# zengxiaofei/HapHiC

Hardware: AMD Instinct MI355X
Metric: Hi-C pairs/s ingested (link-matrix build) + MCL iters/s (higher is better)
Workload: dtype u64 keys + u32 counts (ingest); f32 values, exact u64 fixed-point accumulation (MCL)

## Files before the change

haphic_amd/csrc/hhx_ingest.h:

```cpp
#pragma once
#include "hhx_common.h"
#include "hhx_internal.h"

namespace hhx {

constexpr int ID_BITS = 29;
constexpr u64 ID_MASK = (1ull << ID_BITS) - 1;
constexpr u64 KEY_MASK = (1ull << (2 * ID_BITS)) - 1;
constexpr int HT_SHIFT = 58;
constexpr u64 FULL_BIT = 1ull << 60, FLANK_BIT = 1ull << 61;
constexpr u64 EMPTY_KEY = ~0ull, NO_ORD = ~0ull;

struct LinkRun {
    i64 n = 0;
    DevBuf<u64> key, ord_full, ord_flank;
    DevBuf<u32> ht;
    DevBuf<u32> fl;
    bool has_stats = false;
    unsigned long long stats[3] = {0, 0, 0};
    int alloc(i64 rows) {
        n = rows;
        return key.alloc((size_t)rows) || ord_full.alloc((size_t)rows) || ord_flank.alloc((size_t)rows) ||
               ht.alloc((size_t)rows * 4) || fl.alloc((size_t)rows);
    }
// ... 84 lines not shown
    bool ready = false;
    i64 n_full = 0, n_flank = 0;
    DevBuf<i32> full_i, full_j, flank_i, flank_j;
    DevBuf<i64> full_cnt, ht, flank_cnt;
    DevBuf<double> flank_val;
    DevBuf<unsigned long long> frag_links;
};

}

struct hhx_ingest {
    hhx::DevTables t{};
    hhx::DevBuf<hhx::UnitInfo> ctg_info, frag_info;
    bool combined = true;
    u64 ord_base = 0;
    u64 n_pushed = 0;
    u64 ord_limit = 0;
    std::vector<hhx::LinkRun *> runs[3];
    bool keep_frag_pairs = false;
    bool finalized = false;
    i64 n_full = 0, n_flank = 0;
    hhx::OrderedTables ordered;
    bool keep_pairs = false;
    std::vector<hhx::DevBuf<u64>> side_key, side_xy;
    i64 n_side = 0;
    bool links_dropped = false;
    std::vector<i32> frag_ctg;
    bool pairs_dropped = false;
    i64 max_ctg_len = 0;
    hhx::DevBuf<i32> stage[4];
    hhx::DevBuf<i64> stage64[2];
    ~hhx_ingest() {
        for (auto &v : runs)
            for (auto *r : v) delete r;
    }
    const hhx::LinkRun *table(int which) const {
        const auto &v = runs[(combined || which == 0) ? 0 : 1];
        return v.empty() ? nullptr : v[0];
    }
};

template <class POS>
int hhx_side_records_push(hhx_ingest *h, i64 n_pairs, const i32 *id1, const POS *pos1, const i32 *id2, const POS *pos2);

namespace hhx {
struct PairGroups {
    i64 K = 0, N = 0;
    DevBuf<u64> skey, sxy, stk, srank;
    DevBuf<i64> gstart;
};
int group_pairs(hhx_ingest *h, PairGroups &G, const char *who);
}

int hhx_link_matrix_from_run(const hhx::LinkRun *run, i32 n_frag, u64 ord_limit, const uint8_t *in_set_host, i32 n_rest, int add_self_loops,
                             i32 *frag_index_host, i32 *n_linked_out, hhx_csr **out);

namespace hhx {
int ingest_write_clm_fd(hhx_ingest *h, int fd, const uint8_t *names_blob, const i64 *name_off, i64 *n_lines, i64 *n_bytes);
}
```

haphic_amd/csrc/hhx_ingest.hip:

```cpp
#include "hhx_ingest.h"
#include "hhx_partition.h"

using namespace hhx;

namespace {

__device__ __host__ __forceinline__ u64 mix64(u64 x) {
    x ^= x >> 33; x *= 0xff51afd7ed558ccdULL; x ^= x >> 33; x *= 0xc4ceb9fe1a85ec53ULL; x ^= x >> 33;
    return x;
}
__device__ __forceinline__ u32 bucket_of(u64 key, int total_bits) {
    return total_bits ? (u32)(mix64(key) >> (64 - total_bits)) : 0u;
}

template <bool COMBINED, class POS = i32>
struct SrcPairs {
    typedef u32 w1_t;
    static constexpr bool MARK = false;
    static constexpr bool BATCHED = false;
    const i32 *id1; const POS *pos1; const i32 *id2; const POS *pos2;
    DevTables t;
    int stream;
    __device__ __forceinline__ bool get(i64 idx, u64 &rec, u32 &ord) const {
        ord = (u32)idx;
// ... 763 lines not shown
    if (key) *key = r ? r->key.p : nullptr;
    if (ord_full) *ord_full = r ? r->ord_full.p : nullptr;
    if (ord_flank) *ord_flank = r ? r->ord_flank.p : nullptr;
    if (ht) *ht = r ? r->ht.p : nullptr;
    if (flank) *flank = r ? r->fl.p : nullptr;
    return 0;
}

extern "C" int hhx_ingest_fetch(hhx_ingest *h, i32 *full_i, i32 *full_j, i64 *full_cnt, i64 *ht_cnt, i32 *flank_i, i32 *flank_j,
                                i64 *flank_cnt, i64 *frag_links) {
    if (!h || !h->finalized) return fail("ingest handle not finalized");
    HHX_TRY(materialize(h));
    const OrderedTables &o = h->ordered;
    const size_t nf = (size_t)o.n_full, nk = (size_t)o.n_flank;
    if (full_i && nf) HHX_HIP(hipMemcpyAsync(full_i, o.full_i.p, 4 * nf, hipMemcpyDeviceToHost, g_stream));
    if (full_j && nf) HHX_HIP(hipMemcpyAsync(full_j, o.full_j.p, 4 * nf, hipMemcpyDeviceToHost, g_stream));
    if (full_cnt && nf) HHX_HIP(hipMemcpyAsync(full_cnt, o.full_cnt.p, 8 * nf, hipMemcpyDeviceToHost, g_stream));
    if (ht_cnt && nf) HHX_HIP(hipMemcpyAsync(ht_cnt, o.ht.p, 32 * nf, hipMemcpyDeviceToHost, g_stream));
    if (flank_i && nk) HHX_HIP(hipMemcpyAsync(flank_i, o.flank_i.p, 4 * nk, hipMemcpyDeviceToHost, g_stream));
    if (flank_j && nk) HHX_HIP(hipMemcpyAsync(flank_j, o.flank_j.p, 4 * nk, hipMemcpyDeviceToHost, g_stream));
    if (flank_cnt && nk) HHX_HIP(hipMemcpyAsync(flank_cnt, o.flank_cnt.p, 8 * nk, hipMemcpyDeviceToHost, g_stream));
    if (frag_links) HHX_HIP(hipMemcpyAsync(frag_links, o.frag_links.p, 8 * (size_t)h->t.n_frag, hipMemcpyDeviceToHost, g_stream));
    HHX_HIP(hipStreamSynchronize(g_stream));
    return 0;
}

int hhx_ingest_ordered_full_device(hhx_ingest *h, const i32 **fi, const i32 **fj) {
    HHX_TRY(materialize(h));
    *fi = h->ordered.full_i.p;
    *fj = h->ordered.full_j.p;
    return 0;
}

extern "C" int hhx_ingest_flank_device(hhx_ingest *h, void **fi, void **fj, void **val) {
    if (!h || !h->finalized) return fail("ingest handle not finalized");
    HHX_TRY(materialize(h));
    if (fi) *fi = h->ordered.flank_i.p;
    if (fj) *fj = h->ordered.flank_j.p;
    if (val) *val = h->ordered.flank_val.p;
    return 0;
}

extern "C" int hhx_ingest_flank_count_device(hhx_ingest *h, void **cnt_i64) {
    if (!h || !h->finalized) return fail("ingest handle not finalized");
    HHX_TRY(materialize(h));
    if (cnt_i64) *cnt_i64 = h->ordered.flank_cnt.p;
    return 0;
}

extern "C" int hhx_ingest_link_matrix(hhx_ingest *h, const uint8_t *in_set_host, int32_t n_rest, int add_self_loops,
                                      int32_t *frag_index_host, int32_t *n_linked, hhx_csr **out) {
    if (!h || !h->finalized) return fail("ingest handle not finalized");
    KTimer kt("link_matrix");
    return hhx_link_matrix_from_run(h->table(1), h->t.n_frag, h->ord_limit, in_set_host, n_rest, add_self_loops, frag_index_host, n_linked, out);
}

extern "C" int hhx_ingest_destroy(hhx_ingest *h) {
    if (h) files_wait_handle(h);
    delete h;
    return 0;
}
```

haphic_amd/csrc/hhx_matrix.hip:

```cpp
#include "hhx_ingest.h"
#include "hhx_partition.h"
#include "hhx_sort.h"

using namespace hhx;

namespace {

struct RowsView {
    const i32 *fi, *fj;
    const double *val;
    __device__ __forceinline__ bool get(i64 k, i32 &a, i32 &b, u64 &ord, float &v) const {
        a = fi[k]; b = fj[k]; ord = (u64)k;
        v = (float)val[k];
        return true;
    }
};
struct RunView {
    const u64 *key, *ord_flank;
    const u32 *fl;
    __device__ __forceinline__ bool get(i64 k, i32 &a, i32 &b, u64 &ord, float &v) const {
        ord = ord_flank[k];
        if (ord == NO_ORD) return false;
        a = (i32)(key[k] >> ID_BITS); b = (i32)(key[k] & ID_MASK);
        v = (float)fl[k];
// ... 213 lines not shown
namespace {

struct SrcDirected {
    typedef u64 w1_t;
    static constexpr bool MARK = false;
    static constexpr bool BATCHED = false;
    const u64 *key, *ord_flank;
    const u32 *fl;
    const unsigned char *in_set;
    __device__ __forceinline__ bool get(i64 idx, u64 &w0, u64 &w1) const {
        const i64 k = idx >> 1;
        const u64 ord = ord_flank[k];
        if (ord == NO_ORD) return false;
        const u64 ky = key[k];
        const u32 i = (u32)(ky >> ID_BITS), j = (u32)(ky & ID_MASK);
        if (!in_set[i] || !in_set[j]) return false;
        const u32 side = (u32)(idx & 1);
        const u32 a = side ? j : i, b = side ? i : j;
        w0 = ((u64)a << ID_BITS) | (u64)b;
        w1 = ((2 * ord + side) << 31) | (u64)fl[k];
        return true;
    }
};
struct DigRow {
    __device__ __forceinline__ u32 operator()(u64 w0) const { return (u32)(w0 >> ID_BITS); }
};

constexpr int PK_ID_BITS = 20, PK_CNT_BITS = 24;
constexpr u32 PK_ID_MASK = (1u << PK_ID_BITS) - 1, PK_CNT_MASK = (1u << PK_CNT_BITS) - 1;
__device__ __forceinline__ u32 xcc_id() {
#if defined(__HIP_DEVICE_COMPILE__)
    return __builtin_amdgcn_s_getreg((3 << 11) | 20) & 7u;
#else
    return 0;
#endif
}
constexpr i32 D2M_LDS_MAX_FRAGS = 1 << 19;
struct PackedRawBase { u64 ord, ky; u32 c; };
struct PackedRawWords : PackedRawBase { u32 wi, wj; };
template <bool IN_LDS>
struct SrcDirectedPacked {
    typedef NoPayload w1_t;
    static constexpr bool MARK = true;
    static constexpr bool BATCHED = true;
    static constexpr bool LDS_TABLE = IN_LDS;
    static constexpr size_t LDS_TABLE_MAX = (size_t)D2M_LDS_MAX_FRAGS / 8;
    static constexpr int CHUNK = 7, CHUNK_SCATTER = 4;
    const u64 *key, *ord_flank;
    const u32 *fl;
    const u32 *in_bits;
    unsigned long long *first_pos;
    unsigned int *too_big;
    i32 n_frag;
    typedef typename std::conditional<IN_LDS, PackedRawBase, PackedRawWords>::type Raw;
    static constexpr int PREFETCH = 1;
    static __device__ __forceinline__ void pin(Raw &r) { asm volatile("" : "+v"(r.ord)); asm volatile("" : "+v"(r.ky)); asm volatile("" : "+v"(r.c)); }
    __device__ __forceinline__ u32 frag_i(const Raw &r) const { return min((u32)(r.ky >> ID_BITS), (u32)n_frag - 1u); }
    __device__ __forceinline__ u32 frag_j(const Raw &r) const { return min((u32)(r.ky & ID_MASK), (u32)n_frag - 1u); }
    size_t lds_table_bytes() const { return ((size_t)n_frag + 31) / 32 * sizeof(u32); }
    __device__ __forceinline__ SrcDirectedPacked lds_table(void *at) const {
        u32 *t = (u32 *)at;
        const u32 words = ((u32)n_frag + 31u) >> 5;
        for (u32 w = threadIdx.x; w < words; w += blockDim.x) t[w] = in_bits[w];
        SrcDirectedPacked s = *this;
        s.in_bits = t;
        return s;
    }
    __device__ __forceinline__ void load1(i64 idx, Raw &r) const {
        const i64 k = idx >> 1;
        r.ord = ord_flank[k]; r.ky = key[k]; r.c = fl[k];
    }
    __device__ __forceinline__ void load2(Raw &r) const {
        if constexpr (!IN_LDS) { r.wi = in_bits[frag_i(r) >> 5]; r.wj = in_bits[frag_j(r) >> 5]; }
    }
    __device__ __forceinline__ bool member(const Raw &r) const {
        const u32 fi = frag_i(r), fj = frag_j(r);
        u32 wi, wj;
        if constexpr (IN_LDS) { wi = in_bits[fi >> 5]; wj = in_bits[fj >> 5]; }
        else { wi = r.wi; wj = r.wj; }
        return ((wi >> (fi & 31u)) & (wj >> (fj & 31u)) & 1u) != 0;
    }
    __device__ __forceinline__ bool decode_marked(i64 idx, const Raw &r, u64 &w0, u64 &extra) const {
        const u32 i = (u32)(r.ky >> ID_BITS), j = (u32)(r.ky & ID_MASK);
        const u32 side = (u32)(idx & 1);
        const u32 a = side ? j : i, b = side ? i : j;
        w0 = ((u64)a << (PK_ID_BITS + PK_CNT_BITS)) | ((u64)b << PK_CNT_BITS) | (u64)(r.c & PK_CNT_MASK);
        extra = r.c > PK_CNT_MASK ? ~0ull : 2 * r.ord + side;
        return r.ord != NO_ORD && member(r);
    }
    __device__ __forceinline__ bool decode(i64 idx, const Raw &r, u64 &w0, NoPayload &) const {
        u64 extra;
        return decode_marked(idx, r, w0, extra);
    }
    __device__ __forceinline__ bool get(i64 idx, u64 &w0, NoPayload &w1) const {
        Raw r;
        load1(idx, r);
        load2(r);
        return decode(idx, r, w0, w1);
    }
    __device__ __forceinline__ unsigned long long *my_table() const {
        return first_pos + (size_t)xcc_id() * (size_t)n_frag;
    }
    __device__ __forceinline__ u64 mark_load(i64 idx, const Raw &r) const {
        if (!first_pos) return 0;
        return __hip_atomic_load(&my_table()[(idx & 1) ? frag_j(r) : frag_i(r)], __ATOMIC_RELAXED, __HIP_MEMORY_SCOPE_AGENT);
    }
    __device__ __forceinline__ void mark_apply(u64 w0, u64 pos, u64 seen) const {
        if (!first_pos) return;
        if (pos == ~0ull) *too_big = 1u;
        else if (pos < seen) atomicMin(&my_table()[(u32)(w0 >> (PK_ID_BITS + PK_CNT_BITS)) & PK_ID_MASK], (unsigned long long)pos);
    }
};
constexpr int N_XCC = 8;
__global__ __launch_bounds__(256) void k_min_over_xcc(i32 n_frag, const unsigned long long *__restrict__ per_xcc, unsigned long long *__restrict__ out) {
    for (i32 f = blockIdx.x * blockDim.x + threadIdx.x; f < n_frag; f += gridDim.x * blockDim.x) {
        unsigned long long m = ~0ull;
#pragma unroll
        for (int x = 0; x < N_XCC; ++x) m = min(m, per_xcc[(size_t)x * n_frag + f]);
        out[f] = m;
    }
}
struct DigRowPacked {
    __device__ __forceinline__ u32 operator()(u64 w0) const { return (u32)(w0 >> (PK_ID_BITS + PK_CNT_BITS)) & PK_ID_MASK; }
};
__global__ __launch_bounds__(256) void k_len_from_base(i32 n_frag, const i64 *__restrict__ base, const i32 *__restrict__ frag_index, i32 *__restrict__ cnt) {
    for (i32 f = blockIdx.x * blockDim.x + threadIdx.x; f < n_frag; f += gridDim.x * blockDim.x)
        if (frag_index[f] >= 0) cnt[frag_index[f]] += (i32)(base[f + 1] - base[f]);
}
__global__ __launch_bounds__(256) void k_iota_u64(i64 n, u64 *out) {
    for (i64 k = (i64)blockIdx.x * blockDim.x + threadIdx.x; k < n; k += (i64)gridDim.x * blockDim.x) out[k] = (u64)k;
}
__global__ __launch_bounds__(256) void k_index_from_sorted(i64 n, const u64 *__restrict__ pos_sorted, const u64 *__restrict__ frag_sorted,
                                                           i32 *__restrict__ frag_index, unsigned int *n_linked) {
    for (i64 k = (i64)blockIdx.x * blockDim.x + threadIdx.x; k < n; k += (i64)gridDim.x * blockDim.x) {
        const bool linked = pos_sorted[k] != ~0ull;
        frag_index[frag_sorted[k]] = linked ? (i32)k : -1;
        if (linked && (k + 1 == n || pos_sorted[k + 1] == ~0ull)) *n_linked = (unsigned int)(k + 1);
    }
}
int rank_first_positions(i32 n_frag, const unsigned long long *first_pos, u64 pos_limit, i32 *frag_index, unsigned int *n_linked_dev) {
    if (n_frag <= 4096) {
        k_rank_first<<<(unsigned)((n_frag + 255) / 256), 256, 0, g_stream>>>(n_frag, first_pos, frag_index, n_linked_dev);
        HHX_LAUNCH_CHECK();
        return 0;
    }
    int bits = 1;
    while (bits < 64 && (pos_limit + 1) >> bits) ++bits;
    DevBuf<u64> iota, ks, vs;
    if (iota.alloc((size_t)n_frag) || ks.alloc((size_t)n_frag) || vs.alloc((size_t)n_frag)) return 1;
    k_iota_u64<<<(unsigned)((n_frag + 255) / 256), 256, 0, g_stream>>>(n_frag, iota.p);
    HHX_LAUNCH_CHECK();
    HHX_TRY(stable_sort_pairs_u64((const u64 *)first_pos, ks.p, iota.p, vs.p, n_frag, bits));
    k_index_from_sorted<<<(unsigned)((n_frag + 255) / 256), 256, 0, g_stream>>>(n_frag, ks.p, vs.p, frag_index, n_linked_dev);
    HHX_LAUNCH_CHECK();
    HHX_HIP(hipStreamSynchronize(g_stream));
    return 0;
}

__global__ __launch_bounds__(256) void k_row_first(i32 n_frag, const i64 *__restrict__ base, const u64 *__restrict__ w1,
                                                   unsigned long long *__restrict__ first_pos, i32 *__restrict__ row_len) {
    const int lane = lane_id();
    for (i32 a = blockIdx.x * 4 + threadIdx.x / HHX_WAVE; a < n_frag; a += gridDim.x * 4) {
        const i64 b = base[a], e = base[a + 1];
        unsigned long long m = ~0ull;
        for (i64 p = b + lane; p < e; p += HHX_WAVE) m = min(m, (unsigned long long)(w1[p] >> 31));
#pragma unroll
        for (int o = 32; o > 0; o >>= 1) m = min(m, (unsigned long long)__shfl_down((long long)m, o, HHX_WAVE));
        if (lane == 0) { first_pos[a] = m; row_len[a] = (i32)(e - b); }
    }
}
__global__ __launch_bounds__(256) void k_len_by_index(i32 n_frag, const i32 *__restrict__ frag_index, const i32 *__restrict__ row_len,
                                                      i32 *__restrict__ cnt) {
    for (i32 f = blockIdx.x * blockDim.x + threadIdx.x; f < n_frag; f += gridDim.x * blockDim.x)
        if (frag_index[f] >= 0) cnt[frag_index[f]] += row_len[f];
}
template <bool PACKED>
__device__ __forceinline__ u32 entry_col(u64 w0) { return PACKED ? ((u32)(w0 >> PK_CNT_BITS) & PK_ID_MASK) : (u32)(w0 & ID_MASK); }
template <bool PACKED>
__device__ __forceinline__ float entry_val(u64 w0, const u64 *__restrict__ w1, i64 p) {
    return PACKED ? (float)((u32)w0 & PK_CNT_MASK) : (float)(u32)(w1[p] & 0x7fffffffu);
}
constexpr int EMIT_T = 512, EMIT_R = 8;
constexpr int EMIT_MIN_STAGE = EMIT_T;
template <bool PACKED, bool STAGED>
__global__ __launch_bounds__(EMIT_T) void k_row_emit(i32 n_frag, i32 W, i32 S, int self_loop, const i64 *__restrict__ base, const u64 *__restrict__ w0,
                                                     const u64 *__restrict__ w1, const i32 *__restrict__ frag_index,
                                                     const i32 *__restrict__ indptr, i32 *__restrict__ oj, float *__restrict__ ox) {
    extern __shared__ __attribute__((aligned(16))) unsigned char smem[];
    u32 *bitmap = (u32 *)smem, *prefix = bitmap + W, *wsum = prefix + W;
    i32 *sj = (i32 *)(wsum + EMIT_T / HHX_WAVE);
    float *sx = (float *)(sj + S);
    const int tid = threadIdx.x, lane = lane_id(), wave = tid / HHX_WAVE;
    i32 a = blockIdx.x;
    if (a >= n_frag) return;
    i32 r = frag_index[a];
    i64 b = base[a], e = r < 0 ? b : base[a + 1];
    u64 t0[EMIT_R];
#pragma unroll
    for (int u = 0; u < EMIT_R; ++u) { const i64 p = b + tid + (i64)u * EMIT_T; t0[u] = p < e ? w0[p] : 0; }
#pragma unroll
    for (int u = 0; u < EMIT_R; ++u) asm volatile("" : "+v"(t0[u]));
    for (;;) {
        const i32 an = a + gridDim.x;
        i32 rn = -1;
        i64 bn = 0, en = 0;
        u64 tn[EMIT_R];
        if (an < n_frag) { rn = frag_index[an]; bn = base[an]; en = rn < 0 ? bn : base[an + 1]; }
#pragma unroll
// ... 75 lines not shown
            for (i64 p = b + tid + (i64)EMIT_R * EMIT_T; p < e; p += EMIT_T) {
                const u64 t = w0[p];
                const i32 c = frag_index[entry_col<PACKED>(t)];
                const i32 k = (i32)(prefix[c >> 5] + __popc(bitmap[c >> 5] & ((1u << (c & 31)) - 1u)));
                oj[ob + k] = c;
                ox[ob + k] = entry_val<PACKED>(t, w1, p);
            }
            if (self_loop && tid == 0) {
                const i32 k = (i32)(prefix[r >> 5] + __popc(bitmap[r >> 5] & ((1u << (r & 31)) - 1u)));
                oj[ob + k] = r;
                ox[ob + k] = 1.0f;
            }
            lds_barrier();
            }
        } else {
#pragma unroll
            for (int u = 0; u < EMIT_R; ++u) asm volatile("" : "+v"(tn[u]));
            asm volatile("" : "+v"(rn)); asm volatile("" : "+v"(bn)); asm volatile("" : "+v"(en));
        }
        if (an >= n_frag) break;
        a = an; r = rn; b = bn; e = en;
#pragma unroll
        for (int u = 0; u < EMIT_R; ++u) t0[u] = tn[u];
    }
}
__global__ __launch_bounds__(256) void k_rest_rows(i32 r0, i32 shape, const i32 *__restrict__ indptr, i32 *__restrict__ oj, float *__restrict__ ox) {
    for (i32 r = r0 + blockIdx.x * blockDim.x + threadIdx.x; r < shape; r += gridDim.x * blockDim.x) { oj[indptr[r]] = r; ox[indptr[r]] = 1.0f; }
}

i64 pack_membership(const uint8_t *in_set_host, i32 n_frag, u32 *bits) {
    const i32 n_words = (n_frag + 31) / 32;
    for (i32 w = 0; w < n_words; ++w) bits[w] = 0;
    i64 members = 0;
    i32 f = 0;
    for (; f + 8 <= n_frag; f += 8) {
        u64 x;
        memcpy(&x, in_set_host + f, 8);
        const u64 y = (((x & 0x7f7f7f7f7f7f7f7full) + 0x7f7f7f7f7f7f7f7full) | x) & 0x8080808080808080ull;
        const u32 m = (u32)(((y >> 7) * 0x0102040810204080ull) >> 56);
        bits[f >> 5] |= m << (f & 31);
        members += __builtin_popcount(m);
    }
    for (; f < n_frag; ++f)
        if (in_set_host[f]) { bits[f >> 5] |= 1u << (f & 31); ++members; }
    return members;
}
i32 d2m_lds_frags() {
    const char *e = getenv("HHX_D2M_LDS_FRAGS");
    if (!e || !*e) return D2M_LDS_MAX_FRAGS;
    const long long v = atoll(e);
    return v <= 0 ? 0 : (i32)std::min<long long>(v, D2M_LDS_MAX_FRAGS);
}

size_t emit_stage_cap() {
    const char *e = getenv("HHX_EMIT_STAGE");
    if (!e || !*e) return SIZE_MAX;
    const long long v = atoll(e);
    return v <= 0 ? 0 : (size_t)v;
}
i64 emit_grid_cap() { const char *e = getenv("HHX_EMIT_GRID"); return e && atoll(e) > 0 ? atoll(e) : 0; }
constexpr size_t EMIT_LDS_MAX = 160 * 1024;
constexpr int EMIT_ROUNDS = 3;

template <bool PACKED>
int link_matrix_partitioned(const LinkRun *run, i32 n_frag, u64 ord_limit, const uint8_t *in_set_host, i32 n_rest, int add_self_loops,
                            i32 *frag_index_host, i32 *n_linked_out, hhx_csr **out) {
    typedef typename std::conditional<PACKED, NoPayload, u64>::type W1;
    DevBuf<unsigned char> in_set;
    DevBuf<u32> in_bits;
    std::vector<u32> bits_host;
    i64 members = 0;
    if constexpr (PACKED) {
        bits_host.resize(((size_t)n_frag + 31) / 32);
        members = pack_membership(in_set_host, n_frag, bits_host.data());
        if (in_bits.alloc(bits_host.size())) return 1;
        HHX_HIP(hipMemcpyAsync(in_bits.p, bits_host.data(), sizeof(u32) * bits_host.size(), hipMemcpyHostToDevice, g_stream));
    } else {
        if (in_set.alloc((size_t)n_frag)) return 1;
        HHX_HIP(hipMemcpyAsync(in_set.p, in_set_host, (size_t)n_frag, hipMemcpyHostToDevice, g_stream));
    }
    int row_bits = 0;
    while (((i64)1 << row_bits) < n_frag) ++row_bits;
    DevBuf<unsigned long long> first_pos;
    DevBuf<i32> frag_index, row_len;
    DevBuf<unsigned int> nl;
    if (first_pos.alloc((size_t)n_frag) || frag_index.alloc((size_t)n_frag) || nl.alloc(2)) return 1;
    HHX_HIP(hipMemsetAsync(nl.p, 0, 2 * sizeof(unsigned int), g_stream));
    Partitioned<W1> part;
    static const int level_bits = getenv("HHX_D2M_LBITS") ? atoi(getenv("HHX_D2M_LBITS")) : 9;
    if constexpr (PACKED) {
        DevBuf<unsigned long long> per_xcc;
        if (per_xcc.alloc((size_t)N_XCC * (size_t)n_frag)) return 1;
        HHX_HIP(hipMemsetAsync(per_xcc.p, 0xff, sizeof(unsigned long long) * (size_t)N_XCC * (size_t)n_frag, g_stream));
        if (n_frag <= d2m_lds_frags()) {
            const SrcDirectedPacked<true> src{run->key.p, run->ord_flank.p, run->fl.p, in_bits.p, nullptr, nullptr, n_frag};
            const SrcDirectedPacked<true> marking{run->key.p, run->ord_flank.p, run->fl.p, in_bits.p, per_xcc.p, nl.p + 1, n_frag};
            HHX_TRY(partition_records(src, DigRowPacked(), 2 * run->n, row_bits, level_bits, &part, "d2m", &marking));
        } else {
            const SrcDirectedPacked<false> src{run->key.p, run->ord_flank.p, run->fl.p, in_bits.p, nullptr, nullptr, n_frag};
            const SrcDirectedPacked<false> marking{run->key.p, run->ord_flank.p, run->fl.p, in_bits.p, per_xcc.p, nl.p + 1, n_frag};
            HHX_TRY(partition_records(src, DigRowPacked(), 2 * run->n, row_bits, level_bits, &part, "d2m", &marking));
        }
        k_min_over_xcc<<<grid_for((u64)n_frag), 256, 0, g_stream>>>(n_frag, per_xcc.p, first_pos.p);
        HHX_LAUNCH_CHECK();
    } else {
        const SrcDirected src{run->key.p, run->ord_flank.p, run->fl.p, in_set.p};
        HHX_TRY(partition_records(src, DigRow(), 2 * run->n, row_bits, level_bits, &part, "d2m"));
        if (row_len.alloc((size_t)n_frag)) return 1;
        if (part.n_valid == 0) {
            HHX_HIP(hipMemsetAsync(first_pos.p, 0xff, sizeof(unsigned long long) * (size_t)n_frag, g_stream));
            HHX_HIP(hipMemsetAsync(row_len.p, 0, sizeof(i32) * (size_t)n_frag, g_stream));
        } else {
            KTimer kt("d2m_row_first");
            k_row_first<<<grid_for((u64)n_frag * 64), 256, 0, g_stream>>>(n_frag, part.base.p, part.w1.p, first_pos.p, row_len.p);
        }
        HHX_LAUNCH_CHECK();
    }
    { KTimer kt("d2m_rank");
    HHX_TRY(rank_first_positions(n_frag, first_pos.p, 2 * ord_limit + 1, frag_index.p, nl.p)); }
    unsigned int nl_host[2] = {0, 0};
    HHX_HIP(hipMemcpyAsync(nl_host, nl.p, sizeof nl_host, hipMemcpyDeviceToHost, g_stream));
    if (!PACKED && n_rest < 0)
        for (i32 f = 0; f < n_frag; ++f) members += in_set_host[f] != 0;
    HHX_HIP(hipStreamSynchronize(g_stream));
    if (PACKED && nl_host[1]) return -2;
    const unsigned int n_linked = nl_host[0];
    if (n_rest < 0) n_rest = (i32)(members - (i64)n_linked);
    const i64 shape64 = (i64)n_linked + n_rest;
    if (shape64 > INT32_MAX) return fail("matrix order exceeds int32");
    const i32 shape = (i32)shape64;
    DevBuf<i32> cnt, indptr;
    if (cnt.alloc((size_t)shape + 1) || indptr.alloc((size_t)shape + 2)) return 1;
    k_init_counts<<<grid_for((u64)shape + 1), 256, 0, g_stream>>>(shape, cnt.p, add_self_loops ? 1 : 0);
    if (part.n_valid) {
        if (PACKED) k_len_from_base<<<grid_for((u64)n_frag), 256, 0, g_stream>>>(n_frag, part.base.p, frag_index.p, cnt.p);
        else k_len_by_index<<<grid_for((u64)n_frag), 256, 0, g_stream>>>(n_frag, frag_index.p, row_len.p, cnt.p);
    }
    HHX_LAUNCH_CHECK();
    i64 nnz = 0;
    HHX_TRY(exclusive_scan_i32(cnt.p, indptr.p, shape, &nnz));
    hhx_csr *m = nullptr;
    HHX_TRY(hhx_csr_alloc_internal(shape, shape, nnz, &m));
    hipError_t e = hipMemcpyAsync(m->indptr.p, indptr.p, sizeof(i32) * ((size_t)shape + 1), hipMemcpyDeviceToDevice, g_stream);
    const i32 W = (shape + 31) / 32;
    const size_t lds = (size_t)W * 8 + (EMIT_T / HHX_WAVE) * 4;
    if (lds > EMIT_LDS_MAX) { hhx_csr_free(m); return fail("link matrix: order %d exceeds the LDS bitmap capacity", shape); }
    static int attr_set = -1, n_cu = 0;
    int attr_dev = 0;
    HHX_HIP(hipGetDevice(&attr_dev));
    if (attr_set != attr_dev) {
        (void)hipFuncSetAttribute((const void *)k_row_emit<PACKED, false>, hipFuncAttributeMaxDynamicSharedMemorySize, (int)EMIT_LDS_MAX);
        (void)hipFuncSetAttribute((const void *)k_row_emit<PACKED, true>, hipFuncAttributeMaxDynamicSharedMemorySize, (int)EMIT_LDS_MAX);
        (void)hipDeviceGetAttribute(&n_cu, hipDeviceAttributeMultiprocessorCount, attr_dev);
        attr_set = attr_dev;
    }
    if (e == hipSuccess && part.n_valid) {
        const size_t want = emit_stage_cap();
        int resident = 0;
        (void)hipOccupancyMaxActiveBlocksPerMultiprocessor(&resident, (const void *)k_row_emit<PACKED, true>, EMIT_T, lds);
        if (resident < 1) resident = 1;
        size_t S = want ? (EMIT_LDS_MAX / (size_t)resident > lds ? (EMIT_LDS_MAX / (size_t)resident - lds) / 8 : 0) : 0;
        for (int with = 0; S >= (size_t)EMIT_MIN_STAGE; S -= 64) {
            if (hipOccupancyMaxActiveBlocksPerMultiprocessor(&with, (const void *)k_row_emit<PACKED, true>, EMIT_T, lds + S * 8) != hipSuccess || with >= resident) break;
        }
        if (S < (size_t)EMIT_MIN_STAGE) S = 0;
        else S = std::min(std::min(S, want), (size_t)shape);
        if (!S) (void)hipOccupancyMaxActiveBlocksPerMultiprocessor(&resident, (const void *)k_row_emit<PACKED, false>, EMIT_T, lds);
        i64 grid = std::min<i64>(n_frag, (i64)std::max(resident, 1) * std::max(n_cu, 1) * EMIT_ROUNDS);
        if (const i64 cap = emit_grid_cap()) grid = std::min(grid, cap);
        KTimer kt("d2m_emit");
        if (S)
            k_row_emit<PACKED, true><<<(unsigned)grid, EMIT_T, lds + S * 8, g_stream>>>(n_frag, W, (i32)S, add_self_loops, part.base.p, part.w0.p,
                                                                                      (const u64 *)part.w1.p, frag_index.p, indptr.p, m->indices.p, m->data.p);
        else
            k_row_emit<PACKED, false><<<(unsigned)grid, EMIT_T, lds, g_stream>>>(n_frag, W, 0, add_self_loops, part.base.p, part.w0.p,
                                                                                 (const u64 *)part.w1.p, frag_index.p, indptr.p, m->indices.p, m->data.p);
    }
    if (e == hipSuccess && add_self_loops && shape > (i32)n_linked)
        k_rest_rows<<<grid_for((u64)(shape - (i32)n_linked)), 256, 0, g_stream>>>((i32)n_linked, shape, indptr.p, m->indices.p, m->data.p);
    if (e == hipSuccess) e = hipGetLastError();
    if (e == hipSuccess && frag_index_host)
        e = hipMemcpyAsync(frag_index_host, frag_index.p, sizeof(i32) * (size_t)n_frag, hipMemcpyDeviceToHost, g_stream);
    if (e == hipSuccess) e = hipStreamSynchronize(g_stream);
    if (e != hipSuccess) { hhx_csr_free(m); return fail("link matrix: %s", hipGetErrorString(e)); }
    if (n_linked_out) *n_linked_out = (i32)n_linked;
    *out = m;
    return 0;
}

}

int hhx_link_matrix_from_run(const LinkRun *run, i32 n_frag, u64 ord_limit, const uint8_t *in_set_host, i32 n_rest, int add_self_loops,
                             i32 *frag_index_host, i32 *n_linked_out, hhx_csr **out) {
    if (!out || !in_set_host || n_frag <= 0) return fail("hhx_ingest_link_matrix: bad argument");
    if (run && run->n && n_frag <= (1 << 20) && ord_limit <= ((u64)1 << 31) && !getenv("HHX_D2M_GENERIC")) {
        if (!getenv("HHX_D2M_WIDE")) {
            const int rc = link_matrix_partitioned<true>(run, n_frag, ord_limit, in_set_host, n_rest, add_self_loops, frag_index_host, n_linked_out, out);
            if (rc != -2) return rc;
        }
        return link_matrix_partitioned<false>(run, n_frag, ord_limit, in_set_host, n_rest, add_self_loops, frag_index_host, n_linked_out, out);
    }
    const RunView vw{run ? run->key.p : nullptr, run ? run->ord_flank.p : nullptr, run ? run->fl.p : nullptr};
    return build_matrix(vw, run ? run->n : 0, n_frag, in_set_host, n_rest, add_self_loops, frag_index_host, n_linked_out, out);
}

struct hhx_shard {
    i32 n_frag = 0;
    hhx::Partitioned<u64> part;
    hhx::DevBuf<long long> first;
    hhx::DevBuf<i32> row_len;
    hhx::DevBuf<u64> out_w0, out_w1;
    hhx::DevBuf<unsigned char> in_set;
};

namespace {

constexpr long long SHARD_NONE = INT64_MAX;

__global__ __launch_bounds__(256) void k_first_signed(i32 n_frag, const unsigned long long *__restrict__ first_pos, long long *__restrict__ out) {
    for (i32 f = blockIdx.x * blockDim.x + threadIdx.x; f < n_frag; f += gridDim.x * blockDim.x)
        out[f] = first_pos[f] == ~0ull ? SHARD_NONE : (long long)first_pos[f];
}
__global__ __launch_bounds__(256) void k_len_by_row(i32 n_frag, const i32 *__restrict__ frag_index, const i32 *__restrict__ row_len,
                                                    i64 *__restrict__ len_by_row) {
    for (i32 f = blockIdx.x * blockDim.x + threadIdx.x; f < n_frag; f += gridDim.x * blockDim.x)
        if (frag_index[f] >= 0) len_by_row[frag_index[f]] = row_len[f];
}
__global__ __launch_bounds__(256) void k_emit_by_row(i32 n_frag, const i64 *__restrict__ base, const u64 *__restrict__ w0, const u64 *__restrict__ w1,
                                                     const i32 *__restrict__ frag_index, const i64 *__restrict__ row_off,
                                                     u64 *__restrict__ o0, u64 *__restrict__ o1) {
    const int lane = lane_id();
    for (i32 a = blockIdx.x * 4 + threadIdx.x / HHX_WAVE; a < n_frag; a += gridDim.x * 4) {
        const i32 r = frag_index[a];
        const i64 b = base[a], e = base[a + 1];
        if (r < 0 || b == e) continue;
        const i64 d = row_off[r];
        for (i64 p = b + lane; p < e; p += HHX_WAVE) {
            o0[d + (p - b)] = ((u64)(u32)r << ID_BITS) | (u64)(u32)frag_index[(u32)(w0[p] & ID_MASK)];
            o1[d + (p - b)] = w1[p] & 0x7fffffffull;
        }
    }
}
struct DigLocalRow {
    u32 r0;
    __device__ __forceinline__ u32 operator()(u64 w0) const { return (u32)(w0 >> ID_BITS) - r0; }
};
__device__ __forceinline__ void mark_columns(u32 *bitmap, i32 W, const u64 *__restrict__ w0, i64 b, i64 e, i32 self_col) {
    for (i32 w = threadIdx.x; w < W; w += 256) bitmap[w] = 0;
    __syncthreads();
    for (i64 p = b + threadIdx.x; p < e; p += 256) { const u32 c = (u32)(w0[p] & ID_MASK); atomicOr(&bitmap[c >> 5], 1u << (c & 31)); }
    if (self_col >= 0 && threadIdx.x == 0) atomicOr(&bitmap[self_col >> 5], 1u << (self_col & 31));
    __syncthreads();
}
// ... 338 lines not shown
```

haphic_amd/csrc/hhx_partition.h:

```cpp
#pragma once
#include <type_traits>
#include "hhx_common.h"

namespace hhx {

constexpr int PT = 512, P_MAX_BINS = 512;
struct NoPayload {};
template <class W1> struct PartW1 { static constexpr bool HAS = true; static constexpr size_t BYTES = sizeof(W1); };
template <> struct PartW1<NoPayload> { static constexpr bool HAS = false; static constexpr size_t BYTES = 0; };
template <class W1> struct PartTile { static constexpr int ITEMS = !PartW1<W1>::HAS ? 14 : (sizeof(W1) == 4 ? 8 : 7), TILE = PT * ITEMS; };

struct PartLevel {
    int total_bits;
    int shift;
    int lds_bits;
};

template <class W1>
struct SrcRecs {
    typedef W1 w1_t;
    static constexpr bool MARK = false;
    static constexpr bool BATCHED = true;
    static constexpr int CHUNK = 16, CHUNK_SCATTER = 16, PREFETCH = 2;
    const u64 *w0;
// ... 2 lines not shown
    static __device__ __forceinline__ void pin(Raw &r) {
        asm volatile("" : "+v"(r.a));
        if constexpr (PartW1<W1>::HAS) asm volatile("" : "+v"(r.b));
    }
    __device__ __forceinline__ void load1(i64 idx, Raw &r) const {
        r.a = w0[idx];
        if constexpr (PartW1<W1>::HAS) r.b = w1[idx];
    }
    __device__ __forceinline__ void load2(Raw &) const {}
    __device__ __forceinline__ bool decode(i64, const Raw &r, u64 &a, W1 &b) const {
        a = r.a;
        if constexpr (PartW1<W1>::HAS) b = r.b;
        return true;
    }
    __device__ __forceinline__ bool get(i64 idx, u64 &a, W1 &b) const {
        a = w0[idx];
        if constexpr (PartW1<W1>::HAS) b = w1[idx];
        return true;
    }
};

template <class Src, class = void> struct PartLds { static constexpr bool HAS = false; static constexpr size_t MAX = 0; };
template <class Src> struct PartLds<Src, std::void_t<decltype(Src::LDS_TABLE)>> {
    static constexpr bool HAS = Src::LDS_TABLE;
    static constexpr size_t MAX = HAS ? (Src::LDS_TABLE_MAX + 15) / 16 * 16 : 0;
};
template <class Src> inline size_t part_lds_table_bytes(const Src &src) {
    if constexpr (PartLds<Src>::HAS) return (src.lds_table_bytes() + 15) / 16 * 16;
    else return 0;
}

template <class Src, class Dig>
__device__ __forceinline__ u32 tile_group(const Src &src, const Dig &dig, i64 first, i64 n, const PartLevel &L) {
    if (L.shift + L.lds_bits >= L.total_bits) return 0;
    u64 w0; typename Src::w1_t w1;
    (void)src.get(first < n ? first : n - 1, w0, w1);
    return (dig(w0) >> L.shift) >> L.lds_bits;
}

template <class Src, class Dig>
__global__ __launch_bounds__(PT) void k_part_count(Src src_arg, Dig dig, i64 n, PartLevel L, unsigned long long *__restrict__ ghist) {
    constexpr int P_ITEMS = PartTile<typename Src::w1_t>::ITEMS, P_TILE = PartTile<typename Src::w1_t>::TILE;
    __shared__ u32 hist[P_MAX_BINS];
    __shared__ u32 s_grp;
    extern __shared__ __attribute__((aligned(16))) unsigned char count_smem[];
    const int tid = threadIdx.x, nb = 1 << L.lds_bits;
    for (int t = tid; t < nb; t += PT) hist[t] = 0;
    Src src = src_arg;
    if constexpr (PartLds<Src>::HAS) {
        src = src_arg.lds_table(count_smem);
        lds_barrier();
    }
    u32 cur = 0xffffffffu;
    const i64 n_tiles = (n + P_TILE - 1) / P_TILE;
    for (i64 tile = blockIdx.x; tile < n_tiles; tile += gridDim.x) {
        const i64 base = tile * P_TILE;
        if (tid == 0) s_grp = tile_group(src, dig, base, n, L);
        lds_barrier();
        const u32 tg = s_grp;
        if (tg != cur) {
            if (cur != 0xffffffffu)
                for (int t = tid; t < nb; t += PT) {
                    if (hist[t]) atomicAdd(&ghist[((u64)cur << L.lds_bits) | (u64)t], (unsigned long long)hist[t]);
                    hist[t] = 0;
                }
            cur = tg;
            lds_barrier();
        }
        if constexpr (Src::BATCHED) {
            constexpr int CH = Src::CHUNK < P_ITEMS ? Src::CHUNK : P_ITEMS;
#pragma unroll
            for (int h = 0; h < P_ITEMS; h += CH) {
                typename Src::Raw raw[CH];
                u64 seen[CH];
#pragma unroll
                for (int k = 0; k < CH; ++k)
                    if (h + k < P_ITEMS) {
                        const i64 idx = base + (i64)(h + k) * PT + tid;
                        src.load1(idx < n ? idx : n - 1, raw[k]);
                    }
#pragma unroll
                for (int k = 0; k < CH; ++k)
                    if (h + k < P_ITEMS) {
                        src.load2(raw[k]);
                        if constexpr (Src::MARK) seen[k] = src.mark_load(base + (i64)(h + k) * PT + tid, raw[k]);
                    }
#pragma unroll
                for (int k = 0; k < CH; ++k)
                    if (h + k < P_ITEMS) {
                        const i64 idx = base + (i64)(h + k) * PT + tid;
                        u64 w0, extra = 0;
                        bool ok;
                        if constexpr (Src::MARK) ok = src.decode_marked(idx, raw[k], w0, extra);
                        else { typename Src::w1_t w1; ok = src.decode(idx, raw[k], w0, w1); }
                        if (idx < n && ok) {
                            if constexpr (Src::MARK) src.mark_apply(w0, extra, seen[k]);
                            const u32 d = dig(w0) >> L.shift;
                            if ((d >> L.lds_bits) == tg) atomicAdd(&hist[d & (u32)(nb - 1)], 1u);
                            else atomicAdd(&ghist[d], 1ull);
                        }
                    }
            }
        } else {
            static_assert(!Src::MARK, "a source with a side effect per record is a BATCHED one");
#pragma unroll
        for (int k = 0; k < P_ITEMS; ++k) {
            const i64 idx = base + (i64)k * PT + tid;
            u64 w0; typename Src::w1_t w1;
            if (idx < n && src.get(idx, w0, w1)) {
                const u32 d = dig(w0) >> L.shift;
                if ((d >> L.lds_bits) == tg) atomicAdd(&hist[d & (u32)(nb - 1)], 1u);
                else atomicAdd(&ghist[d], 1ull);
            }
        }
        }
        lds_barrier();
    }
    if (cur != 0xffffffffu)
        for (int t = tid; t < nb; t += PT)
            if (hist[t]) atomicAdd(&ghist[((u64)cur << L.lds_bits) | (u64)t], (unsigned long long)hist[t]);
}

template <class W1, int T>
constexpr size_t part_scatter_lds() {
    return (size_t)PartTile<W1>::ITEMS * T * (8 + PartW1<W1>::BYTES + 2) + (size_t)P_MAX_BINS * (4 + 4 + 8) + 16;
}
template <class W1, int T>
constexpr size_t part_scatter_table_at() { return (part_scatter_lds<W1, T>() + 15) / 16 * 16; }

template <class Src, bool B = Src::BATCHED> struct PartRaw { struct type {}; static constexpr int PF = 0; };
template <class Src> struct PartRaw<Src, true> { typedef typename Src::Raw type; static constexpr int PF = Src::PREFETCH; };

template <class Src, class Dig, int T>
__global__ __launch_bounds__(T) void k_part_scatter(Src src_arg, Dig dig, i64 n, PartLevel L, unsigned long long *__restrict__ cursor,
                                                     u64 *__restrict__ out_w0, typename Src::w1_t *__restrict__ out_w1) {
    typedef typename Src::w1_t W1;
    typedef typename PartRaw<Src>::type RawT;
    constexpr int P_ITEMS = PartTile<W1>::ITEMS, P_TILE = PartTile<W1>::ITEMS * T, PF = PartRaw<Src>::PF;
    static_assert(P_TILE <= 0x10000 && P_MAX_BINS <= 0x8000, "bin and rank of a record share one register");
    extern __shared__ __attribute__((aligned(16))) unsigned char smem[];
    u64 *s_w0 = (u64 *)smem;
    unsigned long long *gbase = (unsigned long long *)(s_w0 + P_TILE);
    W1 *s_w1 = (W1 *)(gbase + P_MAX_BINS);
    u32 *hist = (u32 *)((unsigned char *)s_w1 + (size_t)P_TILE * PartW1<W1>::BYTES);
    u32 *lbase = hist + P_MAX_BINS;
    u32 *s_misc = lbase + P_MAX_BINS;
    unsigned short *s_bin = (unsigned short *)(s_misc + 4);
    const int tid = threadIdx.x, lane = lane_id(), wave = tid / HHX_WAVE, nb = 1 << L.lds_bits;
    __shared__ u32 wsum[T / HHX_WAVE];
    const i64 n_tiles = (n + P_TILE - 1) / P_TILE;
    if ((i64)blockIdx.x >= n_tiles) return;
    const bool later = L.shift + L.lds_bits < L.total_bits;
    for (int t = tid; t < nb; t += T) hist[t] = 0;
    Src src = src_arg;
    if constexpr (PartLds<Src>::HAS) src = src_arg.lds_table(smem + part_scatter_table_at<W1, T>());
    lds_barrier();
    [[maybe_unused]] auto prefetch = [&](const i64 pbase, RawT (&raw)[P_ITEMS], u64 &gw) {
        if constexpr (PF > 0) {
#pragma unroll
            for (int k = 0; k < P_ITEMS; ++k) {
                const i64 idx = pbase + (i64)k * T + tid;
                src.load1(idx < n ? idx : n - 1, raw[k]);
            }
            if constexpr (PF > 1) {
#pragma unroll
                for (int k = 0; k < P_ITEMS; ++k) src.load2(raw[k]);
            }
            if (later) { W1 gw1; (void)src.get(pbase < n ? pbase : n - 1, gw, gw1); }
        }
    };
    [[maybe_unused]] auto pin = [&](RawT (&raw)[P_ITEMS], u64 &gw) {
        if constexpr (PF > 0) {
#pragma unroll
// ... 230 lines not shown
```

Baseline: 18.07 billion.

## Limit first-position marking to an early cut and repair unsettled rows afterwards

```diff
diff --git a/haphic_amd/csrc/hhx_ingest.h b/haphic_amd/csrc/hhx_ingest.h
--- a/haphic_amd/csrc/hhx_ingest.h
+++ b/haphic_amd/csrc/hhx_ingest.h
@@ -160,7 +160,7 @@
 int group_pairs(hhx_ingest *h, PairGroups &G, const char *who);
 }
 
-int hhx_link_matrix_from_run(const hhx::LinkRun *run, i32 n_frag, u64 ord_limit, const uint8_t *in_set_host, i32 n_rest, int add_self_loops,
+int hhx_link_matrix_from_run(const hhx::LinkRun *run, i32 n_frag, u64 ord_base, u64 ord_limit, const uint8_t *in_set_host, i32 n_rest, int add_self_loops,
                              i32 *frag_index_host, i32 *n_linked_out, hhx_csr **out);
 
 namespace hhx {
diff --git a/haphic_amd/csrc/hhx_ingest.hip b/haphic_amd/csrc/hhx_ingest.hip
--- a/haphic_amd/csrc/hhx_ingest.hip
+++ b/haphic_amd/csrc/hhx_ingest.hip
@@ -839,7 +839,7 @@
                                       int32_t *frag_index_host, int32_t *n_linked, hhx_csr **out) {
     if (!h || !h->finalized) return fail("ingest handle not finalized");
     KTimer kt("link_matrix");
-    return hhx_link_matrix_from_run(h->table(1), h->t.n_frag, h->ord_limit, in_set_host, n_rest, add_self_loops, frag_index_host, n_linked, out);
+    return hhx_link_matrix_from_run(h->table(1), h->t.n_frag, h->ord_base, h->ord_limit, in_set_host, n_rest, add_self_loops, frag_index_host, n_linked, out);
 }
 
 extern "C" int hhx_ingest_destroy(hhx_ingest *h) {
diff --git a/haphic_amd/csrc/hhx_matrix.hip b/haphic_amd/csrc/hhx_matrix.hip
--- a/haphic_amd/csrc/hhx_matrix.hip
+++ b/haphic_amd/csrc/hhx_matrix.hip
@@ -289,6 +289,9 @@
     unsigned long long *first_pos;
     unsigned int *too_big;
     i32 n_frag;
+    u64 cut_pos = ~0ull;
+    u32 park_mask = 0;
+    unsigned long long *n_reads = nullptr;
     typedef typename std::conditional<IN_LDS, PackedRawBase, PackedRawWords>::type Raw;
     static constexpr int PREFETCH = 1;
     static __device__ __forceinline__ void pin(Raw &r) { asm volatile("" : "+v"(r.ord)); asm volatile("" : "+v"(r.ky)); asm volatile("" : "+v"(r.c)); }
@@ -340,12 +343,25 @@
     }
     __device__ __forceinline__ u64 mark_load(i64 idx, const Raw &r) const {
         if (!first_pos) return 0;
-        return __hip_atomic_load(&my_table()[(idx & 1) ? frag_j(r) : frag_i(r)], __ATOMIC_RELAXED, __HIP_MEMORY_SCOPE_AGENT);
-    }
-    __device__ __forceinline__ void mark_apply(u64 w0, u64 pos, u64 seen) const {
+        const u32 side = (u32)(idx & 1);
+        const u32 f = side ? frag_j(r) : frag_i(r);
+        const u32 at = 2 * r.ord + side < cut_pos ? f : ((u32)idx & park_mask);
+        return __hip_atomic_load(&my_table()[at], __ATOMIC_RELAXED, __HIP_MEMORY_SCOPE_AGENT);
+    }
+    __device__ __forceinline__ void mark_apply(u64 w0, u64 pos, u64 seen, u32 &reads) const {
         if (!first_pos) return;
         if (pos == ~0ull) *too_big = 1u;
-        else if (pos < seen) atomicMin(&my_table()[(u32)(w0 >> (PK_ID_BITS + PK_CNT_BITS)) & PK_ID_MASK], (unsigned long long)pos);
+        else if (pos < cut_pos) {
+            ++reads;
+            if (pos < seen) atomicMin(&my_table()[(u32)(w0 >> (PK_ID_BITS + PK_CNT_BITS)) & PK_ID_MASK], (unsigned long long)pos);
+        }
+    }
+    __device__ __forceinline__ void mark_flush(u32 reads) const {
+        if (!first_pos) return;
+        u32 s = reads;
+#pragma unroll
+        for (int o = HHX_WAVE / 2; o > 0; o >>= 1) s += __shfl_down(s, o, HHX_WAVE);
+        if (lane_id() == 0 && s) atomicAdd(n_reads, (unsigned long long)s);
     }
 };
 constexpr int N_XCC = 8;
@@ -360,6 +376,30 @@
 struct DigRowPacked {
     __device__ __forceinline__ u32 operator()(u64 w0) const { return (u32)(w0 >> (PK_ID_BITS + PK_CNT_BITS)) & PK_ID_MASK; }
 };
+__global__ __launch_bounds__(256) void k_first_unsettled(i32 n_frag, const unsigned long long *__restrict__ first_pos, const i64 *__restrict__ base,
+                                                         u32 *__restrict__ bits, unsigned int *__restrict__ n_unsettled) {
+    for (i32 f0 = blockIdx.x * blockDim.x; f0 < n_frag; f0 += gridDim.x * blockDim.x) {
+        const i32 f = f0 + threadIdx.x;
+        const bool un = f < n_frag && first_pos[f] == ~0ull && base[f + 1] > base[f];
+        if (un) atomicOr(&bits[f >> 5], 1u << (f & 31));
+        const unsigned long long m = __ballot(un);
+        if (lane_id() == 0 && m) atomicAdd(n_unsettled, (unsigned int)__popcll(m));
+    }
+}
+__global__ __launch_bounds__(256) void k_first_repair(SrcDirectedPacked<false> src, i64 n, const u32 *__restrict__ bits,
+                                                      const unsigned int *__restrict__ n_unsettled, unsigned long long *first_pos) {
+    if (*n_unsettled == 0) return;
+    for (i64 idx = (i64)blockIdx.x * blockDim.x + threadIdx.x; idx < n; idx += (i64)gridDim.x * blockDim.x) {
+        SrcDirectedPacked<false>::Raw r;
+        src.load1(idx, r);
+        src.load2(r);
+        u64 w0, pos;
+        if (!src.decode_marked(idx, r, w0, pos) || pos == ~0ull) continue;
+        const u32 row = DigRowPacked()(w0);
+        if (!((bits[row >> 5] >> (row & 31u)) & 1u)) continue;
+        if (pos < __hip_atomic_load(&first_pos[row], __ATOMIC_RELAXED, __HIP_MEMORY_SCOPE_AGENT)) atomicMin(&first_pos[row], (unsigned long long)pos);
+    }
+}
 __global__ __launch_bounds__(256) void k_len_from_base(i32 n_frag, const i64 *__restrict__ base, const i32 *__restrict__ frag_index, i32 *__restrict__ cnt) {
     for (i32 f = blockIdx.x * blockDim.x + threadIdx.x; f < n_frag; f += gridDim.x * blockDim.x)
         if (frag_index[f] >= 0) cnt[frag_index[f]] += (i32)(base[f + 1] - base[f]);
@@ -375,7 +415,8 @@
         if (linked && (k + 1 == n || pos_sorted[k + 1] == ~0ull)) *n_linked = (unsigned int)(k + 1);
     }
 }
-int rank_first_positions(i32 n_frag, const unsigned long long *first_pos, u64 pos_limit, i32 *frag_index, unsigned int *n_linked_dev) {
+struct RankBufs { DevBuf<u64> iota, ks, vs; };
+int rank_first_positions(i32 n_frag, const unsigned long long *first_pos, u64 pos_limit, i32 *frag_index, unsigned int *n_linked_dev, RankBufs &bufs) {
     if (n_frag <= 4096) {
         k_rank_first<<<(unsigned)((n_frag + 255) / 256), 256, 0, g_stream>>>(n_frag, first_pos, frag_index, n_linked_dev);
         HHX_LAUNCH_CHECK();
@@ -383,14 +424,12 @@
     }
     int bits = 1;
     while (bits < 64 && (pos_limit + 1) >> bits) ++bits;
-    DevBuf<u64> iota, ks, vs;
-    if (iota.alloc((size_t)n_frag) || ks.alloc((size_t)n_frag) || vs.alloc((size_t)n_frag)) return 1;
-    k_iota_u64<<<(unsigned)((n_frag + 255) / 256), 256, 0, g_stream>>>(n_frag, iota.p);
+    if (bufs.iota.alloc((size_t)n_frag) || bufs.ks.alloc((size_t)n_frag) || bufs.vs.alloc((size_t)n_frag)) return 1;
+    k_iota_u64<<<(unsigned)((n_frag + 255) / 256), 256, 0, g_stream>>>(n_frag, bufs.iota.p);
     HHX_LAUNCH_CHECK();
-    HHX_TRY(stable_sort_pairs_u64((const u64 *)first_pos, ks.p, iota.p, vs.p, n_frag, bits));
-    k_index_from_sorted<<<(unsigned)((n_frag + 255) / 256), 256, 0, g_stream>>>(n_frag, ks.p, vs.p, frag_index, n_linked_dev);
+    HHX_TRY(stable_sort_pairs_u64((const u64 *)first_pos, bufs.ks.p, bufs.iota.p, bufs.vs.p, n_frag, bits));
+    k_index_from_sorted<<<(unsigned)((n_frag + 255) / 256), 256, 0, g_stream>>>(n_frag, bufs.ks.p, bufs.vs.p, frag_index, n_linked_dev);
     HHX_LAUNCH_CHECK();
-    HHX_HIP(hipStreamSynchronize(g_stream));
     return 0;
 }
 
@@ -572,6 +611,15 @@
     return v <= 0 ? 0 : (i32)std::min<long long>(v, D2M_LDS_MAX_FRAGS);
 }
 
+constexpr u64 D2M_FIRST_CUT_DIV = 16;
+u64 d2m_first_cut_pos(u64 ord_base, u64 ord_limit) {
+    const char *e = getenv("HHX_D2M_FIRST_CUT");
+    const u64 span = ord_limit > ord_base ? ord_limit - ord_base : 0;
+    const u64 count = e && *e ? (u64)strtoull(e, nullptr, 10) : (span + D2M_FIRST_CUT_DIV - 1) / D2M_FIRST_CUT_DIV;
+    if (count >= ((u64)1 << 62) || ord_base >= ((u64)1 << 62)) return ~0ull;
+    return 2 * (ord_base + count);
+}
+
 size_t emit_stage_cap() {
     const char *e = getenv("HHX_EMIT_STAGE");
     if (!e || !*e) return SIZE_MAX;
@@ -583,7 +631,7 @@
 constexpr int EMIT_ROUNDS = 3;
 
 template <bool PACKED>
-int link_matrix_partitioned(const LinkRun *run, i32 n_frag, u64 ord_limit, const uint8_t *in_set_host, i32 n_rest, int add_self_loops,
+int link_matrix_partitioned(const LinkRun *run, i32 n_frag, u64 ord_base, u64 ord_limit, const uint8_t *in_set_host, i32 n_rest, int add_self_loops,
                             i32 *frag_index_host, i32 *n_linked_out, hhx_csr **out) {
     typedef typename std::conditional<PACKED, NoPayload, u64>::type W1;
     DevBuf<unsigned char> in_set;
@@ -603,26 +651,45 @@
     while (((i64)1 << row_bits) < n_frag) ++row_bits;
     DevBuf<unsigned long long> first_pos;
     DevBuf<i32> frag_index, row_len;
-    DevBuf<unsigned int> nl;
-    if (first_pos.alloc((size_t)n_frag) || frag_index.alloc((size_t)n_frag) || nl.alloc(2)) return 1;
-    HHX_HIP(hipMemsetAsync(nl.p, 0, 2 * sizeof(unsigned int), g_stream));
+    struct Words { unsigned int n_linked, too_big, unsettled, pad; unsigned long long reads; };
+    DevBuf<Words> nl_buf;
+    DevBuf<u32> unsettled_bits;
+    if (first_pos.alloc((size_t)n_frag) || frag_index.alloc((size_t)n_frag) || nl_buf.alloc(1)) return 1;
+    HHX_HIP(hipMemsetAsync(nl_buf.p, 0, sizeof(Words), g_stream));
+    unsigned int *const nl = &nl_buf.p->n_linked;
     Partitioned<W1> part;
     static const int level_bits = getenv("HHX_D2M_LBITS") ? atoi(getenv("HHX_D2M_LBITS")) : 9;
     if constexpr (PACKED) {
         DevBuf<unsigned long long> per_xcc;
         if (per_xcc.alloc((size_t)N_XCC * (size_t)n_frag)) return 1;
         HHX_HIP(hipMemsetAsync(per_xcc.p, 0xff, sizeof(unsigned long long) * (size_t)N_XCC * (size_t)n_frag, g_stream));
+        const u64 cut_pos = d2m_first_cut_pos(ord_base, ord_limit);
+        u32 park = 1;
+        while ((u64)park * 2 <= (u64)n_frag) park *= 2;
         if (n_frag <= d2m_lds_frags()) {
             const SrcDirectedPacked<true> src{run->key.p, run->ord_flank.p, run->fl.p, in_bits.p, nullptr, nullptr, n_frag};
-            const SrcDirectedPacked<true> marking{run->key.p, run->ord_flank.p, run->fl.p, in_bits.p, per_xcc.p, nl.p + 1, n_frag};
+            const SrcDirectedPacked<true> marking{run->key.p, run->ord_flank.p, run->fl.p, in_bits.p, per_xcc.p, &nl_buf.p->too_big, n_frag,
+                                                  cut_pos, park - 1, &nl_buf.p->reads};
             HHX_TRY(partition_records(src, DigRowPacked(), 2 * run->n, row_bits, level_bits, &part, "d2m", &marking));
         } else {
             const SrcDirectedPacked<false> src{run->key.p, run->ord_flank.p, run->fl.p, in_bits.p, nullptr, nullptr, n_frag};
-            const SrcDirectedPacked<false> marking{run->key.p, run->ord_flank.p, run->fl.p, in_bits.p, per_xcc.p, nl.p + 1, n_frag};
+            const SrcDirectedPacked<false> marking{run->key.p, run->ord_flank.p, run->fl.p, in_bits.p, per_xcc.p, &nl_buf.p->too_big, n_frag,
+                                                   cut_pos, park - 1, &nl_buf.p->reads};
             HHX_TRY(partition_records(src, DigRowPacked(), 2 * run->n, row_bits, level_bits, &part, "d2m", &marking));
         }
         k_min_over_xcc<<<grid_for((u64)n_frag), 256, 0, g_stream>>>(n_frag, per_xcc.p, first_pos.p);
         HHX_LAUNCH_CHECK();
+        if (part.n_valid && cut_pos != ~0ull) {
+            KTimer kt("d2m_first_repair");
+            const size_t n_words = ((size_t)n_frag + 31) / 32;
+            if (unsettled_bits.alloc(n_words)) return 1;
+            HHX_HIP(hipMemsetAsync(unsettled_bits.p, 0, sizeof(u32) * n_words, g_stream));
+            k_first_unsettled<<<grid_for((u64)n_frag), 256, 0, g_stream>>>(n_frag, first_pos.p, part.base.p, unsettled_bits.p, &nl_buf.p->unsettled);
+            HHX_LAUNCH_CHECK();
+            const SrcDirectedPacked<false> again{run->key.p, run->ord_flank.p, run->fl.p, in_bits.p, nullptr, nullptr, n_frag};
+            k_first_repair<<<grid_for((u64)(2 * run->n)), 256, 0, g_stream>>>(again, 2 * run->n, unsettled_bits.p, &nl_buf.p->unsettled, first_pos.p);
+            HHX_LAUNCH_CHECK();
+        }
     } else {
         const SrcDirected src{run->key.p, run->ord_flank.p, run->fl.p, in_set.p};
         HHX_TRY(partition_records(src, DigRow(), 2 * run->n, row_bits, level_bits, &part, "d2m"));
@@ -636,15 +703,21 @@
         }
         HHX_LAUNCH_CHECK();
     }
+    RankBufs rank_bufs;
     { KTimer kt("d2m_rank");
-    HHX_TRY(rank_first_positions(n_frag, first_pos.p, 2 * ord_limit + 1, frag_index.p, nl.p)); }
-    unsigned int nl_host[2] = {0, 0};
-    HHX_HIP(hipMemcpyAsync(nl_host, nl.p, sizeof nl_host, hipMemcpyDeviceToHost, g_stream));
+    HHX_TRY(rank_first_positions(n_frag, first_pos.p, 2 * ord_limit + 1, frag_index.p, nl, rank_bufs)); }
+    Words nl_host{};
+    HHX_HIP(hipMemcpyAsync(&nl_host, nl_buf.p, sizeof nl_host, hipMemcpyDeviceToHost, g_stream));
     if (!PACKED && n_rest < 0)
         for (i32 f = 0; f < n_frag; ++f) members += in_set_host[f] != 0;
     HHX_HIP(hipStreamSynchronize(g_stream));
-    if (PACKED && nl_host[1]) return -2;
-    const unsigned int n_linked = nl_host[0];
+    rank_bufs = RankBufs();
+    if (PACKED && nl_host.too_big) return -2;
+    if (PACKED) {
+        prof_count("d2m_first_unsettled", (i64)nl_host.unsettled);
+        prof_count("d2m_first_reads", (i64)nl_host.reads);
+    }
+    const unsigned int n_linked = nl_host.n_linked;
     if (n_rest < 0) n_rest = (i32)(members - (i64)n_linked);
     const i64 shape64 = (i64)n_linked + n_rest;
     if (shape64 > INT32_MAX) return fail("matrix order exceeds int32");
@@ -710,15 +783,15 @@
 
 }
 
-int hhx_link_matrix_from_run(const LinkRun *run, i32 n_frag, u64 ord_limit, const uint8_t *in_set_host, i32 n_rest, int add_self_loops,
+int hhx_link_matrix_from_run(const LinkRun *run, i32 n_frag, u64 ord_base, u64 ord_limit, const uint8_t *in_set_host, i32 n_rest, int add_self_loops,
                              i32 *frag_index_host, i32 *n_linked_out, hhx_csr **out) {
     if (!out || !in_set_host || n_frag <= 0) return fail("hhx_ingest_link_matrix: bad argument");
     if (run && run->n && n_frag <= (1 << 20) && ord_limit <= ((u64)1 << 31) && !getenv("HHX_D2M_GENERIC")) {
         if (!getenv("HHX_D2M_WIDE")) {
-            const int rc = link_matrix_partitioned<true>(run, n_frag, ord_limit, in_set_host, n_rest, add_self_loops, frag_index_host, n_linked_out, out);
+            const int rc = link_matrix_partitioned<true>(run, n_frag, ord_base, ord_limit, in_set_host, n_rest, add_self_loops, frag_index_host, n_linked_out, out);
             if (rc != -2) return rc;
         }
-        return link_matrix_partitioned<false>(run, n_frag, ord_limit, in_set_host, n_rest, add_self_loops, frag_index_host, n_linked_out, out);
+        return link_matrix_partitioned<false>(run, n_frag, ord_base, ord_limit, in_set_host, n_rest, add_self_loops, frag_index_host, n_linked_out, out);
     }
     const RunView vw{run ? run->key.p : nullptr, run ? run->ord_flank.p : nullptr, run ? run->fl.p : nullptr};
     return build_matrix(vw, run ? run->n : 0, n_frag, in_set_host, n_rest, add_self_loops, frag_index_host, n_linked_out, out);
diff --git a/haphic_amd/csrc/hhx_partition.h b/haphic_amd/csrc/hhx_partition.h
--- a/haphic_amd/csrc/hhx_partition.h
+++ b/haphic_amd/csrc/hhx_partition.h
@@ -78,6 +78,7 @@
         lds_barrier();
     }
     u32 cur = 0xffffffffu;
+    u32 marked = 0;
     const i64 n_tiles = (n + P_TILE - 1) / P_TILE;
     for (i64 tile = blockIdx.x; tile < n_tiles; tile += gridDim.x) {
         const i64 base = tile * P_TILE;
@@ -120,7 +121,7 @@
                         if constexpr (Src::MARK) ok = src.decode_marked(idx, raw[k], w0, extra);
                         else { typename Src::w1_t w1; ok = src.decode(idx, raw[k], w0, w1); }
                         if (idx < n && ok) {
-                            if constexpr (Src::MARK) src.mark_apply(w0, extra, seen[k]);
+                            if constexpr (Src::MARK) src.mark_apply(w0, extra, seen[k], marked);
                             const u32 d = dig(w0) >> L.shift;
                             if ((d >> L.lds_bits) == tg) atomicAdd(&hist[d & (u32)(nb - 1)], 1u);
                             else atomicAdd(&ghist[d], 1ull);
@@ -145,6 +146,7 @@
     if (cur != 0xffffffffu)
         for (int t = tid; t < nb; t += PT)
             if (hist[t]) atomicAdd(&ghist[((u64)cur << L.lds_bits) | (u64)t], (unsigned long long)hist[t]);
+    if constexpr (Src::MARK) src.mark_flush(marked);
 }
 
 template <class W1, int T>
```

Result: faster. 19.01 billion, median of 6 (+5.2%).
